# talmolab/track-mjx

Measured on AMD Instinct MI355X. Metric: env-steps/sec (whole node), rodent task @ 4096 envs/GPU, higher is better.
Workload: dtype f32

## Files before the change

### include/tmjx.h

```cpp
#ifndef TMJX_H
#define TMJX_H
#include <stddef.h>
#include <stdint.h>

#ifdef __cplusplus
extern "C" {
#endif

#define TMJX_OK 0
#define TMJX_EINVAL (-22)
#define TMJX_ENOMEM (-12)
#define TMJX_EHIP (-5)

typedef struct tmjx_model tmjx_model;

typedef struct tmjx_layout_t {
  int32_t nq, nv, nu, nbody, ncon, nefc, obs_size, ref_obs_size, n_metrics, window;
  int32_t qpos, qvel, act, qacc_warmstart, time;
  int32_t xpos, xmat_torso, qfrc_actuator;
  int32_t prev_ctrl, action_buffer, done, steps_f;
  int32_t first_phys, first_obs, first_prev_ctrl;
  int32_t state_rows;
  int32_t i_clip_idx, i_start_frame, i_buffer_index, i_nan_count, istate_rows;
  int32_t ws_rows;
// ... 42 lines not shown
int tmjx_gae(const float *truncation, const float *termination, const float *rewards, const float *values,
             const float *bootstrap, float lambda_, float discount, float *vs, float *advantages, int T, int B,
             void *stream);

typedef struct {
  int32_t T, B, A, Z;
  float reward_scaling, discounting, gae_lambda, clip_eps, entropy_cost, kl_weight;
  int32_t normalize_advantage;
  int32_t accumulate;
} tmjx_ppo_cfg_t;
int tmjx_ppo_scratch_floats(int T, int B);
int tmjx_ppo_loss(const tmjx_ppo_cfg_t *cfg, const float *logits, const float *raw_action, const float *behaviour_logp,
                  const float *noise, const float *baseline, const float *bootstrap, const float *reward, const float *discount,
                  const float *truncation, const float *fc2, float *dlogits, float *dbaseline, float *dfc2, float *scratch,
                  float *out, void *stream);

#define TMJX_PPO_PHASE_A 1
#define TMJX_PPO_PHASE_B 2
#define TMJX_PPO_PHASE_C 4
#define TMJX_PPO_PHASE_D 8
int tmjx_ppo_loss_phases(const tmjx_ppo_cfg_t *cfg, const float *logits, const float *raw_action, const float *behaviour_logp,
                         const float *noise, const float *baseline, const float *bootstrap, const float *reward, const float *discount,
                         const float *truncation, const float *fc2, float *dlogits, float *dbaseline, float *dfc2, float *scratch,
                         float *out, int phases, void *stream);

int tmjx_silu_ln_partial_floats(int rows, int H);
int tmjx_silu_ln_fwd(const float *z, const float *bias, const float *gamma, const float *beta, float *y, float *stats, int rows, int H,
                     float eps, void *stream);
int tmjx_silu_ln_bwd(const float *dy, const float *z, const float *bias, const float *gamma, const float *stats, float *dz, float *grads,
                     float *partial, int rows, int H, void *stream);
int tmjx_silu_ln_fwd_bf16(const float *z, const float *bias, const float *gamma, const float *beta, uint16_t *y16, int ldy16, float *stats, int rows, int H,
                          float eps, void *stream);
int tmjx_silu_ln_bwd_bf16(const float *dy, const float *z, const float *bias, const float *gamma, const float *stats, uint16_t *dz16, int lddz16, float *grads,
                          float *partial, int rows, int H, void *stream);

int tmjx_gather_normalize(const float *src, const int64_t *idx, const float *mean, const float *std, float *out, int T, int R, int B,
                          int W, void *stream);
int tmjx_gather_minibatch(const float *obs, const float *next_last, const float *raw_action, const float *log_prob, const float *reward, const float *discount,
                          const float *truncation, const int64_t *idx, const float *mean, const float *std, float *obs_n, float *next_n, float *raw_action_g,
                          float *scalars_g, int T, int R, int B, int W, int A, void *stream);
#define TMJX_MINIBATCH_STATE_WORDS (16 + 16 * 64)
typedef struct tmjx_minibatch_t {
  const float *obs, *next_last, *raw_action, *log_prob, *reward, *discount, *truncation;
  const int64_t *perm;
  const float *mean, *std;
  float *obs_n, *next_n, *raw_action_g, *scalars_g;
  float *eps, *noise;
  int64_t *state;
  uint64_t seed;
  int32_t T, R, B, W, A, Z, advance;
} tmjx_minibatch_t;
int tmjx_minibatch_begin(const tmjx_minibatch_t *mb, void *stream);
int tmjx_minibatch_begin_bf16(const tmjx_minibatch_t *mb, uint16_t *obs_n16, int ld16, void *stream);
int tmjx_philox4x32_10(const uint32_t *ctr_key_dev, uint32_t *out_dev, void *stream);

int tmjx_latent_concat_bwd(const float *dx, const float *eps, const float *fc2, float *dfc2, int n, int Z, int dx_stride, void *stream);
int tmjx_latent_concat_bwd_add(const float *dx, const float *eps, const float *fc2, const float *add, float *dfc2, int n, int Z, int dx_stride,
                               void *stream);

int tmjx_latent_concat(const float *fc2, const float *eps, const float *obs, float *x, int n, int Z, int obs_w, int ref_w,
                       int64_t obs_s0, int64_t obs_s1, const float *mean, const float *std, int x_stride, uint64_t seed, const int64_t *rng_state,
                       void *stream);
int tmjx_sample_action(const float *logits, const float *noise, float *raw, float *action_t, float *logp, int n, int A, uint64_t seed,
                       int64_t *rng_state, void *stream);

int tmjx_linear_act_ok(const float *A, int64_t lda, const float *W, int ldw, int K);
int tmjx_linear_act(const float *A, int64_t lda, const float *W, int ldw, const float *bias, float *C, int M, int N, int K,
                    const float *mean, const float *inv_std, void *stream);
int tmjx_linear_nolds(const float *A, int64_t sa_row, int64_t sa_k, const float *W, const float *bias, float *C, int M, int N, int K,
                      void *stream);
int tmjx_linear_nolds_norm(const float *A, int64_t sa_row, int64_t sa_k, const float *W, const float *bias, float *C, int M, int N, int K,
                           const float *mean, const float *inv_std, void *stream);

int tmjx_linear_nolds_bf16(const float *A, int64_t sa_row, int64_t sa_k, const uint16_t *W, int ldw, const float *bias, float *C, int M, int N, int K,
                           const float *mean, const float *inv_std, void *stream);

int tmjx_colsum_scratch_floats(int width);
int tmjx_colsum(const float *src, float *out, float *scratch, int rows, int width, void *stream);

typedef struct tmjx_colsum_problem_t { const float *partial; float *out; int32_t rows, width; } tmjx_colsum_problem_t;
int tmjx_colsum_grouped(const tmjx_colsum_problem_t *problems, int n, void *stream);

int tmjx_adam_clip(float *param, const float *grad, float *exp_avg, float *exp_avg_sq, const float *grad_norm, long long n, float lr,
                   float beta1, float beta2, float eps, float bias_correction1, float bias_correction2, float max_norm, void *stream);
int tmjx_adam_norm_floats(void);
int tmjx_adam_clip_norm(float *param, const float *grad, float *exp_avg, float *exp_avg_sq, float *norm_scratch, float *norm_out, long long n, float lr,
                        float beta1, float beta2, float eps, float bias_correction1, float bias_correction2, float max_norm, void *stream);
int tmjx_adam_clip_norm_frozen(float *param, const float *grad, float *exp_avg, float *exp_avg_sq, float *norm_scratch, float *norm_out, long long n,
                               long long frozen_lo, long long frozen_hi, float lr, float beta1, float beta2, float eps, float bias_correction1,
                               float bias_correction2, float max_norm, void *stream);

int tmjx_gemm_nt(const float *A, int lda, const float *W, int ldw, const float *bias, float *C, int ldc, int M, int N, int K, void *stream);
int tmjx_gemm_nn(const float *A, int lda, const float *W, int ldw, float *C, int ldc, int M, int N, int K, void *stream);
int tmjx_gemm_nt_silu_ln_ok(const float *A, int lda, const float *W, int ldw, int N);
int tmjx_gemm_nt_silu_ln(const float *A, int lda, const float *W, int ldw, const float *bias, const float *gamma, const float *beta, float *Z, float *Y,
                         int ldc, float *stats, int M, int N, int K, float eps, void *stream);
int tmjx_gemm_nn_ln_bwd_ok(const float *dY, int ldy, const float *W, int ldw, int N);
long long tmjx_gemm_nn_ln_bwd_partial_floats(int M, int N);
int tmjx_gemm_nn_ln_bwd(const float *dY, int ldy, const float *W, int ldw, const float *z, const float *bias, const float *gamma, const float *stats,
                        float *dz, float *partial, int M, int N, int K, void *stream);
int tmjx_gemm_nt_silu_ok(const float *A, int lda, const float *W, int ldw);
int tmjx_gemm_nt_silu(const float *A, int lda, const float *W, int ldw, const float *bias, float *Z, float *Y, int ldc, int M, int N, int K, void *stream);
int tmjx_silu_fwd(const float *z, const float *bias, float *y, long long rows, int N, void *stream);
int tmjx_silu_bwd(const float *dy, const float *z, const float *bias, float *dz, long long rows, int N, void *stream);
int tmjx_gemm_nn_silu_bwd_ok(const float *dY, int ldy, const float *W, int ldw);
int tmjx_gemm_nn_silu_bwd(const float *dY, int ldy, const float *W, int ldw, const float *z, const float *bias, float *dZ, int M, int N, int K, void *stream);
// ... 323 lines not shown
```

### track_mjx_amd/csrc/ppo_kernels.h

```cpp
#pragma once
#include "silu_math.h"
#include "act_shared.h"
#include <hip/hip_runtime.h>
#include <math.h>

struct PpoCfg {
  int T, B, A, Z;
  float reward_scaling, discounting, gae_lambda, clip_eps, entropy_cost, kl_weight;
  int normalize_advantage;
  int accumulate;
};

#define PPO_BLOCK 256
#define PPO_ALPHA 0.95f
__device__ __forceinline__ float ppo_sigmoid(float x) { return 1.f / (1.f + expf(-x)); }

template <int NV>
__device__ __forceinline__ void ppo_block_sum(float *v, float *lds) {
  const int tid = threadIdx.x, lane = tid & 63, w = tid >> 6, nw = (blockDim.x + 63) >> 6;
#pragma unroll
  for (int k = 0; k < NV; k++) {
    float x = v[k];
    for (int off = 32; off >= 1; off >>= 1) x += __shfl_xor(x, off);
    if (lane == 0) lds[k * 16 + w] = x;
// ... 668 lines not shown
  const size_t q_eps = g.eps ? ((size_t)g.T * g.B * g.Z + 3) / 4 : 0, q_noise = g.noise ? (n_act + 3) / 4 : 0;
  const size_t e0 = n_obs + n_next, e1 = e0 + n_act, e2 = e1 + n_sc, e3 = e2 + q_eps, total = e3 + q_noise;
  for (size_t i = (size_t)blockIdx.x * 256 + threadIdx.x; i < total; i += (size_t)gridDim.x * 256) {
    if (i < e0) {
      const bool nx = i >= n_obs;
      const size_t j = nx ? i - n_obs : i;
      const int c = (int)(j % w4);
      const size_t tb = j / w4;
      const int b = (int)(tb % g.B), t = (int)(tb / g.B);
      const float *src = nx ? g.next_last : g.obs;
      const float4 v = reinterpret_cast<const float4 *>(src + ((size_t)t * g.R + (size_t)idx[b]) * g.W)[c];
      const float4 m = reinterpret_cast<const float4 *>(g.mean)[c], s = reinterpret_cast<const float4 *>(g.stdv)[c];
      const float4 o = {(v.x - m.x) / s.x, (v.y - m.y) / s.y, (v.z - m.z) / s.z, (v.w - m.w) / s.w};
      reinterpret_cast<float4 *>((nx ? g.next_n : g.obs_n) + tb * g.W)[c] = o;
      if (!nx && g.obs_n16) *reinterpret_cast<uint2 *>(g.obs_n16 + tb * g.ld16 + 4 * c) = uint2{silu_ln_pack(o.x, o.y), silu_ln_pack(o.z, o.w)};
    } else if (i < e1) {
      const size_t j = i - e0;
      const int c = (int)(j % g.A);
      const size_t tb = j / g.A;
      const int b = (int)(tb % g.B), t = (int)(tb / g.B);
      g.raw_action_g[j] = g.raw_action[((size_t)t * g.R + (size_t)idx[b]) * g.A + c];
    } else if (i < e2) {
      const size_t j = i - e1;
      const int b = (int)(j % g.B);
      const size_t kt = j / g.B;
      const int t = (int)(kt % g.T), k = (int)(kt / g.T);
      g.scalars_g[j] = g.scalar[k][(size_t)t * g.R + (size_t)idx[b]];
    } else {
      const bool second = i >= e3;
      const size_t q = second ? i - e3 : i - e2, n = second ? n_act : (size_t)g.T * g.B * g.Z;
      float v[4];
      tm_normal4(g.seed, ctr, second ? 1u : 0u, (unsigned)q, v);
      float *dst = second ? g.noise : g.eps;
#pragma unroll
      for (int k = 0; k < 4; k++) if (4 * q + k < n) dst[4 * q + k] = v[k];
    }
  }
  if (g.state && g.advance) {
    __syncthreads();
    if (threadIdx.x == 0) {
      const unsigned sub = blockIdx.x % TM_MB_SUBTICKETS, nsub = min((unsigned)gridDim.x, (unsigned)TM_MB_SUBTICKETS);
      const unsigned members = (gridDim.x - sub + TM_MB_SUBTICKETS - 1) / TM_MB_SUBTICKETS;
      unsigned long long *st = (unsigned long long *)g.state, *subt = st + TM_MB_STATE_HEAD + (size_t)TM_MB_STATE_STRIDE * sub;
      if (__hip_atomic_fetch_add(subt, 1ull, __ATOMIC_RELAXED, __HIP_MEMORY_SCOPE_AGENT) == (unsigned long long)members - 1ull) {
        __hip_atomic_store(subt, 0ull, __ATOMIC_RELAXED, __HIP_MEMORY_SCOPE_AGENT);
        if (__hip_atomic_fetch_add(st + 2, 1ull, __ATOMIC_RELAXED, __HIP_MEMORY_SCOPE_AGENT) == (unsigned long long)nsub - 1ull) {
          __hip_atomic_store(st + 2, 0ull, __ATOMIC_RELAXED, __HIP_MEMORY_SCOPE_AGENT);
          g.state[0] += 1; g.state[1] += 1;
        }
      }
    }
  }
}
__global__ void k_philox_kat(const unsigned *ctr_key, unsigned *out) {
  if (threadIdx.x == 0) tm_philox4x32_10(ctr_key[0], ctr_key[1], ctr_key[2], ctr_key[3], ctr_key[4], ctr_key[5], out);
}

__global__ __launch_bounds__(256) void k_latent_concat(const float *__restrict__ fc2, const float *__restrict__ eps, const float *__restrict__ obs,
                                                       float *__restrict__ x, int n, int Z, int obs_w, int ref_w, long long obs_s0, long long obs_s1,
                                                       const float *__restrict__ mean, const float *__restrict__ stdv, int x_stride,
                                                       unsigned long long seed, const long long *__restrict__ rng_state) {
  TM_PRIO_ACTING();
  const int W = Z + obs_w - ref_w;
  const unsigned long long ctr = rng_state ? (unsigned long long)rng_state[0] : 0ull;
  for (size_t i = (size_t)blockIdx.x * blockDim.x + threadIdx.x; i < (size_t)n * x_stride; i += (size_t)gridDim.x * blockDim.x) {
    int c = (int)(i % x_stride); size_t e = i / x_stride;
    float v = 0.f;
    if (c < Z) {
      v = tm_latent_sample(tm_normal_at(eps, seed, ctr, 2u, e * Z + c), fc2[e * 2 * Z + Z + c], fc2[e * 2 * Z + c]);
    } else if (c < W) { int k = ref_w + c - Z; v = obs[(long long)e * obs_s0 + (long long)k * obs_s1]; if (mean) v = tm_obs_normalised(v, mean[k], stdv[k]); }
    x[e * (size_t)x_stride + c] = v;
  }
}
__global__ __launch_bounds__(256) void k_latent_concat_bwd(const float *__restrict__ dx, const float *__restrict__ eps, const float *__restrict__ fc2,
                                                           float *__restrict__ dfc2, int n, int Z, int dx_stride, const float *__restrict__ add) {
  for (size_t i = (size_t)blockIdx.x * 256 + threadIdx.x; i < (size_t)n * Z; i += (size_t)gridDim.x * 256) {
    int c = (int)(i % Z); size_t e = i / Z;
    float g = dx[e * (size_t)dx_stride + c];
    float gm = g, gv = g * eps[e * Z + c] * (0.5f * expf(0.5f * fc2[e * 2 * Z + Z + c]));
    if (add) { gm = add[e * 2 * Z + c] + gm; gv = add[e * 2 * Z + Z + c] + gv; }
    dfc2[e * 2 * Z + c] = gm;
    dfc2[e * 2 * Z + Z + c] = gv;
  }
}
__global__ __launch_bounds__(PPO_BLOCK) void k_sample_action(const float *__restrict__ logits, const float *__restrict__ noise, float *__restrict__ raw,
                                                             float *__restrict__ action_t, float *__restrict__ logp, int n, int A,
                                                             unsigned long long seed, long long *__restrict__ rng_state) {
  TM_PRIO_ACTING();
  const int gid = blockIdx.x * blockDim.x + threadIdx.x, e = gid / PPO_G, sub = gid % PPO_G;
  const unsigned long long ctr = rng_state ? (unsigned long long)rng_state[0] : 0ull;
  float lp = 0.f;
  if (e < n) lp = sample_action_lane(logits + (size_t)e * 2 * A, noise, raw, action_t, n, A, (size_t)e, sub, seed, ctr);
  lp = ppo_group_sum(lp);
  if (e < n && sub == 0) logp[e] = lp;
  if (rng_state) {
    __syncthreads();
    if (threadIdx.x == 0) {
      unsigned long long *st = (unsigned long long *)rng_state;
      if (__hip_atomic_fetch_add(st + 1, 1ull, __ATOMIC_RELAXED, __HIP_MEMORY_SCOPE_AGENT) == (unsigned long long)gridDim.x - 1ull) {
        __hip_atomic_store(st + 1, 0ull, __ATOMIC_RELAXED, __HIP_MEMORY_SCOPE_AGENT);
        rng_state[0] += 1;
      }
    }
  }
}

// ... 375 lines not shown
```

### track_mjx_amd/csrc/tmjx_hip.hip

```cpp
#include <hip/hip_runtime.h>

#include <stdlib.h>

#include <string>
#include <vector>

#include "../../include/tmjx.h"
#include "env_core.h"
#include "host_launch.h"
#include "model_host.h"
#include "wave_physics.h"
#ifdef TMJX_LANE_IMPL
#include "../../tests/lane/physics_core.h"
#endif

struct tmjx_model {
  DModel h;
  DModel *d = nullptr;
  float *clips[7] = {nullptr, nullptr, nullptr, nullptr, nullptr, nullptr, nullptr};
  int block = 64;
  int wave = 1;
  bool rodent = false;
  mutable float *mspill = nullptr;
  mutable int mspill_envs = 0;
// ... 708 lines not shown
  switch (H) { case 64: TMJX_FWD(1); break; case 128: TMJX_FWD(2); break; case 256: TMJX_FWD(4); break; case 512: TMJX_FWD(8); break;
               case 1024: TMJX_FWD(16); break; default: return fail(TMJX_EINVAL, "H must be 64, 128, 256, 512 or 1024"); }
#undef TMJX_FWD
  return check_launch("k_silu_ln_fwd");
}
int tmjx_silu_ln_fwd(const float *z, const float *bias, const float *gamma, const float *beta, float *y, float *stats, int rows, int H,
                     float eps, void *stream) {
  if (!y) return fail(TMJX_EINVAL, "null argument");
  return silu_ln_fwd_any(z, bias, gamma, beta, y, nullptr, 0, stats, rows, H, eps, stream);
}
int tmjx_silu_ln_fwd_bf16(const float *z, const float *bias, const float *gamma, const float *beta, uint16_t *y16, int ldy16, float *stats, int rows, int H,
                          float eps, void *stream) {
  if (!y16) return fail(TMJX_EINVAL, "null argument");
  return silu_ln_fwd_any(z, bias, gamma, beta, nullptr, y16, ldy16, stats, rows, H, eps, stream);
}

static int silu_ln_bwd_any(const float *dy, const float *z, const float *bias, const float *gamma, const float *stats, float *dz, uint16_t *dz16, int lddz16, float *grads,
                           float *partial, int rows, int H, void *stream) {
  if (!dy || !z || !bias || !gamma || !stats || (!dz && !dz16) || !grads || !partial) return fail(TMJX_EINVAL, "null argument");
  if (rows < 1) return fail(TMJX_EINVAL, "rows must be >= 1");
  if (dz16 && (lddz16 < H || (lddz16 & 3) || ((uintptr_t)dz16 & 7))) return fail(TMJX_EINVAL, "tmjx_silu_ln_bwd_bf16: the output's rows must be 8-byte aligned and H wide");
  hipStream_t s = (hipStream_t)stream;
  const int nblk = (rows + BLK_ROWS_PER_BLOCK - 1) / BLK_ROWS_PER_BLOCK;
  unsigned short *o16 = (unsigned short *)dz16;
#define TMJX_BWD(V) do { if (o16) hipLaunchKernelGGL((k_silu_ln_bwd<V, true>), dim3(nblk), dim3(256), 0, s, dy, z, bias, gamma, stats, dz, partial, rows, o16, lddz16); \
                         else hipLaunchKernelGGL((k_silu_ln_bwd<V, false>), dim3(nblk), dim3(256), 0, s, dy, z, bias, gamma, stats, dz, partial, rows, o16, 0); } while (0)
  switch (H) { case 64: TMJX_BWD(1); break; case 128: TMJX_BWD(2); break; case 256: TMJX_BWD(4); break; case 512: TMJX_BWD(8); break;
               case 1024: TMJX_BWD(16); break; default: return fail(TMJX_EINVAL, "H must be 64, 128, 256, 512 or 1024"); }
#undef TMJX_BWD
  hipLaunchKernelGGL(k_colsum, dim3((3 * H + 31) / 32), dim3(256), 0, s, (const float *)partial, grads, nblk, 3 * H);
  return check_launch("k_silu_ln_bwd");
}
int tmjx_silu_ln_bwd(const float *dy, const float *z, const float *bias, const float *gamma, const float *stats, float *dz, float *grads,
                     float *partial, int rows, int H, void *stream) {
  if (!dz) return fail(TMJX_EINVAL, "null argument");
  return silu_ln_bwd_any(dy, z, bias, gamma, stats, dz, nullptr, 0, grads, partial, rows, H, stream);
}
int tmjx_silu_ln_bwd_bf16(const float *dy, const float *z, const float *bias, const float *gamma, const float *stats, uint16_t *dz16, int lddz16, float *grads,
                          float *partial, int rows, int H, void *stream) {
  if (!dz16) return fail(TMJX_EINVAL, "null argument");
  return silu_ln_bwd_any(dy, z, bias, gamma, stats, nullptr, dz16, lddz16, grads, partial, rows, H, stream);
}

int tmjx_gather_normalize(const float *src, const int64_t *idx, const float *mean, const float *std, float *out, int T, int R, int B,
                          int W, void *stream) {
  if (!src || !idx || !mean || !std || !out) return fail(TMJX_EINVAL, "null argument");
  if (T < 1 || R < 1 || B < 1 || W < 4 || (W & 3)) return fail(TMJX_EINVAL, "bad T / R / B / W (W must be a multiple of 4)");
  size_t total = (size_t)T * B * (W >> 2);
  int grid = (int)((total + 255) / 256 < 8192 ? (total + 255) / 256 : 8192);
  hipLaunchKernelGGL(k_gather_normalize, dim3(grid), dim3(256), 0, (hipStream_t)stream, src, (const long long *)idx, mean, std, out, T, R, B, W);
  return check_launch("k_gather_normalize");
}

static int launch_minibatch(const MinibatchGather &g, hipStream_t s) {
  if (!g.obs || !g.next_last || !g.raw_action || !g.scalar[0] || !g.scalar[1] || !g.scalar[2] || !g.scalar[3] || !g.idx || !g.mean || !g.stdv || !g.obs_n || !g.next_n ||
      !g.raw_action_g || !g.scalars_g)
    return fail(TMJX_EINVAL, "null argument");
  if (g.T < 1 || g.R < 1 || g.B < 1 || g.A < 1 || g.W < 4 || (g.W & 3)) return fail(TMJX_EINVAL, "bad T / R / B / A / W (W must be a multiple of 4)");
  if (g.eps && g.Z < 1) return fail(TMJX_EINVAL, "Z must be >= 1 with eps");
  const size_t nact = (size_t)g.T * g.B * g.A;
  const size_t total = (size_t)g.T * g.B * (g.W >> 2) + (size_t)g.B * (g.W >> 2) + nact + (size_t)4 * g.T * g.B + (g.eps ? ((size_t)g.T * g.B * g.Z + 3) / 4 : 0) +
                       (g.noise ? (nact + 3) / 4 : 0);
  const int grid = (int)((total + 255) / 256 < 8192 ? (total + 255) / 256 : 8192);
  hipLaunchKernelGGL(k_gather_minibatch, dim3(grid), dim3(256), 0, s, g);
  return check_launch("k_gather_minibatch");
}
int tmjx_gather_minibatch(const float *obs, const float *next_last, const float *raw_action, const float *log_prob, const float *reward, const float *discount,
                          const float *truncation, const int64_t *idx, const float *mean, const float *std, float *obs_n, float *next_n, float *raw_action_g,
                          float *scalars_g, int T, int R, int B, int W, int A, void *stream) {
  MinibatchGather g{obs, next_last, raw_action, {log_prob, reward, discount, truncation}, (const long long *)idx, mean, std, obs_n, next_n, raw_action_g, scalars_g,
                    nullptr, nullptr, nullptr, 0ull, T, R, B, W, A, 0, 0, nullptr, 0};
  return launch_minibatch(g, (hipStream_t)stream);
}
int tmjx_minibatch_begin(const tmjx_minibatch_t *m, void *stream) {
  if (!m) return fail(TMJX_EINVAL, "null argument");
  if ((m->eps || m->noise || m->advance) && !m->state) return fail(TMJX_EINVAL, "tmjx_minibatch_begin: draws / advance need the device state");
  MinibatchGather g{m->obs, m->next_last, m->raw_action, {m->log_prob, m->reward, m->discount, m->truncation}, (const long long *)m->perm, m->mean, m->std, m->obs_n,
                    m->next_n, m->raw_action_g, m->scalars_g, m->eps, m->noise, (long long *)m->state, (unsigned long long)m->seed, m->T, m->R, m->B, m->W, m->A,
                    m->Z, m->advance, nullptr, 0};
  return launch_minibatch(g, (hipStream_t)stream);
}
int tmjx_minibatch_begin_bf16(const tmjx_minibatch_t *m, uint16_t *obs_n16, int ld16, void *stream) {
  if (!m || !obs_n16) return fail(TMJX_EINVAL, "null argument");
  if ((m->eps || m->noise || m->advance) && !m->state) return fail(TMJX_EINVAL, "tmjx_minibatch_begin_bf16: draws / advance need the device state");
  if (ld16 < m->W || (ld16 & 3) || ((uintptr_t)obs_n16 & 7)) return fail(TMJX_EINVAL, "tmjx_minibatch_begin_bf16: the twin's rows must be 8-byte aligned and W wide");
  MinibatchGather g{m->obs, m->next_last, m->raw_action, {m->log_prob, m->reward, m->discount, m->truncation}, (const long long *)m->perm, m->mean, m->std, m->obs_n,
                    m->next_n, m->raw_action_g, m->scalars_g, m->eps, m->noise, (long long *)m->state, (unsigned long long)m->seed, m->T, m->R, m->B, m->W, m->A,
                    m->Z, m->advance, (unsigned short *)obs_n16, ld16};
  return launch_minibatch(g, (hipStream_t)stream);
}
int tmjx_philox4x32_10(const uint32_t *ctr_key_dev, uint32_t *out_dev, void *stream) {
  if (!ctr_key_dev || !out_dev) return fail(TMJX_EINVAL, "null argument");
  hipLaunchKernelGGL(k_philox_kat, dim3(1), dim3(64), 0, (hipStream_t)stream, ctr_key_dev, out_dev);
  return check_launch("k_philox_kat");
}

int tmjx_colsum_scratch_floats(int width) { return COLSUM_CHUNKS * width; }

int tmjx_colsum(const float *src, float *out, float *scratch, int rows, int width, void *stream) {
  if (!src || !out || !scratch) return fail(TMJX_EINVAL, "null argument");
  if (rows < 1 || width < 1) return fail(TMJX_EINVAL, "rows and width must be >= 1");
  hipStream_t s = (hipStream_t)stream;
  hipLaunchKernelGGL(k_colsum_rows, dim3((width + 31) / 32, COLSUM_CHUNKS), dim3(256), 0, s, src, scratch, rows, width);
  hipLaunchKernelGGL(k_colsum, dim3((width + 31) / 32), dim3(256), 0, s, (const float *)scratch, out, COLSUM_CHUNKS, width);
  return check_launch("k_colsum_rows");
}

int tmjx_colsum_grouped(const tmjx_colsum_problem_t *q, int n, void *stream) {
  if (!q || n < 1 || n > COLSUM_GROUP_MAX) return fail(TMJX_EINVAL, "tmjx_colsum_grouped: 1 .. 16 problems");
  ColsumGroup G;
  G.n = n;
  int blocks = 0;
  for (int i = 0; i < n; i++) {
    if (!q[i].partial || !q[i].out || q[i].rows < 1 || q[i].width < 1) return fail(TMJX_EINVAL, "tmjx_colsum_grouped: bad problem");
    G.p[i] = ColsumProblem{q[i].partial, q[i].out, q[i].rows, q[i].width, blocks};
    blocks += (q[i].width + 31) / 32;
  }
  hipLaunchKernelGGL(k_colsum_grouped, dim3(blocks), dim3(256), 0, (hipStream_t)stream, G);
  return check_launch("k_colsum_grouped");
}

int tmjx_adam_clip(float *param, const float *grad, float *exp_avg, float *exp_avg_sq, const float *grad_norm, long long n, float lr,
                   float beta1, float beta2, float eps, float bias_correction1, float bias_correction2, float max_norm, void *stream) {
  if (!param || !grad || !exp_avg || !exp_avg_sq || !grad_norm) return fail(TMJX_EINVAL, "null argument");
  if (n < 1 || !(bias_correction1 > 0.f) || !(bias_correction2 > 0.f) || !(max_norm > 0.f)) return fail(TMJX_EINVAL, "bad n / bias corrections / max_norm");
  int grid = (int)((n + 255) / 256 < 4096 ? (n + 255) / 256 : 4096);
  hipLaunchKernelGGL(k_adam_clip<false>, dim3(grid), dim3(256), 0, (hipStream_t)stream, param, grad, exp_avg, exp_avg_sq, grad_norm, n, lr, beta1, beta2, eps,
                     bias_correction1, bias_correction2, max_norm, (float *)nullptr);
  return check_launch("k_adam_clip");
}
int tmjx_adam_norm_floats(void) { return ADAM_NORM_PARTS; }
int tmjx_adam_clip_norm(float *param, const float *grad, float *exp_avg, float *exp_avg_sq, float *norm_scratch, float *norm_out, long long n, float lr,
                        float beta1, float beta2, float eps, float bias_correction1, float bias_correction2, float max_norm, void *stream) {
  if (!param || !grad || !exp_avg || !exp_avg_sq || !norm_scratch) return fail(TMJX_EINVAL, "null argument");
  if (n < 1 || !(bias_correction1 > 0.f) || !(bias_correction2 > 0.f) || !(max_norm > 0.f)) return fail(TMJX_EINVAL, "bad n / bias corrections / max_norm");
  if ((uintptr_t)grad & 15) return fail(TMJX_EINVAL, "tmjx_adam_clip_norm: the gradient buffer must be 16-byte aligned");
  hipStream_t s = (hipStream_t)stream;
  hipLaunchKernelGGL(k_grad_sumsq, dim3(ADAM_NORM_PARTS), dim3(256), 0, s, grad, n, norm_scratch);
  int grid = (int)((n + 255) / 256 < 4096 ? (n + 255) / 256 : 4096);
  hipLaunchKernelGGL(k_adam_clip<true>, dim3(grid), dim3(256), 0, s, param, grad, exp_avg, exp_avg_sq, (const float *)norm_scratch, n, lr, beta1, beta2, eps,
                     bias_correction1, bias_correction2, max_norm, norm_out);
  return check_launch("k_adam_clip(norm)");
// ... 437 lines not shown
```

### track_mjx_amd/hip.py

```python
from __future__ import annotations

import ctypes as C
import os
import subprocess
from pathlib import Path

_PKG = Path(__file__).resolve().parent
SO_PATH = Path(os.environ.get("TMJX_SO", str(_PKG / "libtmjx_hip.so")))
CSRC = _PKG / "csrc"
SOURCES = (CSRC / "tmjx_hip.hip", CSRC / "tmjx_bf16.hip", CSRC / "tmjx_wave.hip", CSRC / "tmjx_chain.hip", CSRC / "tmjx_lstm.hip",
           CSRC / "tmjx_rollout.hip", CSRC / "tmjx_wave_sensors.hip", CSRC / "tmjx_wave_align.hip", CSRC / "tmjx_wave_rand.hip", CSRC / "tmjx_render.hip", CSRC / "tmjx_act.hip", CSRC / "tmjx_pca.hip", CSRC / "tmjx_pca_wide.hip", CSRC / "tmjx_readout.hip", CSRC / "tmjx_intervene.hip", CSRC / "tmjx_kmeans.hip", CSRC / "tmjx_hmm.hip", CSRC / "tmjx_spectrogram.hip", CSRC / "tmjx_arhmm.hip")
SOURCE_FLAGS = {"tmjx_wave.hip": ("-mllvm", "-disable-machine-licm"),
                "tmjx_wave_sensors.hip": ("-mllvm", "-disable-machine-licm"),
                "tmjx_wave_rand.hip": ("-mllvm", "-disable-machine-licm")}


class TmjxError(RuntimeError):
    pass


class Layout(C.Structure):
    _fields_ = [(n, C.c_int32) for n in (
        "nq", "nv", "nu", "nbody", "ncon", "nefc", "obs_size", "ref_obs_size", "n_metrics", "window",
        "qpos", "qvel", "act", "qacc_warmstart", "time", "xpos", "xmat_torso", "qfrc_actuator",
# ... 146 lines not shown

class ArhmmInfo(C.Structure):
    _fields_ = HmmInfo._fields_ + [("n_singular", C.c_int32), ("pad_", C.c_int32)]


INTERVENE_SUBSPACE, INTERVENE_UNITS, INTERVENE_MAX_W, INTERVENE_MAX_K = 0, 1, 1024, 16


class Intervene(C.Structure):
    _fields_ = [("h", C.c_void_p), ("ld", C.c_int32), ("w", C.c_int32), ("n", C.c_int32), ("mode", C.c_int32), ("dirs", C.c_void_p), ("K", C.c_int32),
                ("ldv", C.c_int32), ("center", C.c_void_p), ("gain", C.c_void_p), ("offset", C.c_void_p), ("dose", C.c_void_p), ("t_on", C.c_void_p),
                ("t_off", C.c_void_p), ("proj", C.c_void_p), ("ldp", C.c_int32), ("pad_", C.c_int32)]


class PcaInfo(C.Structure):
    _fields_ = [("sweeps", C.c_int32), ("converged", C.c_int32), ("off_rel", C.c_float), ("moments_ms", C.c_float), ("jacobi_ms", C.c_float)]


class StripStyle(C.Structure):
    _fields_ = [(k, C.c_int32) for k in ("margin_left", "margin_right", "margin_top", "margin_bottom")] + \
               [("line_half_width", C.c_float), ("marker_radius", C.c_float), ("colour", (C.c_uint8 * 4) * 8)] + \
               [(k, C.c_uint8 * 4) for k in ("background", "axes", "terminated")]


class PpoCfg(C.Structure):
    _fields_ = [("T", C.c_int32), ("B", C.c_int32), ("A", C.c_int32), ("Z", C.c_int32), ("reward_scaling", C.c_float),
                ("discounting", C.c_float), ("gae_lambda", C.c_float), ("clip_eps", C.c_float), ("entropy_cost", C.c_float),
                ("kl_weight", C.c_float), ("normalize_advantage", C.c_int32), ("accumulate", C.c_int32)]


_i, _i64, _u64, _f, _d, _vp, _s, _P = C.c_int, C.c_int64, C.c_uint64, C.c_float, C.c_double, C.c_void_p, C.c_char_p, C.POINTER
SIGNATURES = {
    "tmjx_model_create": ([_s, C.c_size_t, _P(_vp)], _i),
    "tmjx_model_destroy": ([_vp], None),
    "tmjx_layout": ([_vp, _P(Layout)], _i),
    "tmjx_clips_upload": ([_vp] * 6 + [_i, _i], _i),
    "tmjx_reset": ([_vp] * 9 + [_i, _vp], _i),
    "tmjx_step": ([_vp] * 10 + [_i, _vp], _i),
    "tmjx_physics": ([_vp, _vp, _vp, _i, _vp, _i, _vp], _i),
    "tmjx_physics_step": ([_vp] * 4 + [_i, _vp], _i),
    "tmjx_forward": ([_vp, _vp, _vp, _i, _vp], _i),
    "tmjx_reward_obs": ([_vp] * 10 + [_i, _vp], _i),
    "tmjx_reward_frame": ([_vp] * 14 + [_i, _vp], _i),
    "tmjx_gae": ([_vp] * 5 + [_f, _f, _vp, _vp, _i, _i, _vp], _i),
    "tmjx_ppo_scratch_floats": ([_i, _i], _i),
    "tmjx_ppo_loss": ([_P(PpoCfg)] + [_vp] * 16, _i),
    "tmjx_ppo_loss_phases": ([_P(PpoCfg)] + [_vp] * 15 + [_i, _vp], _i),
    "tmjx_silu_ln_partial_floats": ([_i, _i], _i),
    "tmjx_silu_ln_fwd": ([_vp] * 6 + [_i, _i, _f, _vp], _i),
    "tmjx_silu_ln_bwd": ([_vp] * 8 + [_i, _i, _vp], _i),
    "tmjx_silu_ln_fwd_bf16": ([_vp] * 5 + [_i, _vp, _i, _i, _f, _vp], _i),
    "tmjx_silu_ln_bwd_bf16": ([_vp] * 6 + [_i, _vp, _vp, _i, _i, _vp], _i),
    "tmjx_minibatch_begin_bf16": ([_P(Minibatch), _vp, _i, _vp], _i),
    "tmjx_gather_normalize": ([_vp] * 5 + [_i] * 4 + [_vp], _i),
    "tmjx_latent_concat": ([_vp] * 4 + [_i] * 4 + [_i64, _i64, _vp, _vp, _i, _u64, _vp, _vp], _i),
    "tmjx_latent_concat_bwd": ([_vp] * 4 + [_i, _i, _i, _vp], _i),
    "tmjx_latent_concat_bwd_add": ([_vp] * 5 + [_i, _i, _i, _vp], _i),
    "tmjx_sample_action": ([_vp] * 5 + [_i, _i, _u64, _vp, _vp], _i),
    "tmjx_linear_nolds": ([_vp, _i64, _i64, _vp, _vp, _vp, _i, _i, _i, _vp], _i),
    "tmjx_linear_act": ([_vp, _i64, _vp, _i, _vp, _vp, _i, _i, _i, _vp, _vp, _vp], _i),
    "tmjx_linear_act_ok": ([_vp, _i64, _vp, _i, _i], _i),
    "tmjx_linear_nolds_norm": ([_vp, _i64, _i64, _vp, _vp, _vp, _i, _i, _i, _vp, _vp, _vp], _i),
    "tmjx_linear_nolds_bf16": ([_vp, _i64, _i64, _vp, _i, _vp, _vp, _i, _i, _i, _vp, _vp, _vp], _i),
    "tmjx_adam_clip": ([_vp] * 5 + [_i64] + [_f] * 7 + [_vp], _i),
    "tmjx_adam_clip_norm": ([_vp] * 6 + [_i64] + [_f] * 7 + [_vp], _i),
    "tmjx_adam_clip_norm_frozen": ([_vp] * 6 + [_i64, _i64, _i64] + [_f] * 7 + [_vp], _i),
    "tmjx_adam_norm_floats": ([], _i),
    "tmjx_colsum_scratch_floats": ([_i], _i),
    "tmjx_colsum": ([_vp, _vp, _vp, _i, _i, _vp], _i),
    "tmjx_gather_minibatch": ([_vp] * 14 + [_i] * 5 + [_vp], _i),
    "tmjx_minibatch_begin": ([_P(Minibatch), _vp], _i),
    "tmjx_philox4x32_10": ([_vp, _vp, _vp], _i),
    "tmjx_gemm_nt": ([_vp, _i, _vp, _i, _vp, _vp] + [_i] * 4 + [_vp], _i),
    "tmjx_gemm_nt_silu_ln": ([_vp, _i, _vp, _i] + [_vp] * 5 + [_i, _vp, _i, _i, _i, _f, _vp], _i),
    "tmjx_gemm_nt_silu_ln_ok": ([_vp, _i, _vp, _i, _i], _i),
    "tmjx_gemm_nn": ([_vp, _i, _vp, _i, _vp] + [_i] * 4 + [_vp], _i),
    "tmjx_colsum_grouped": ([_P(ColsumProblem), _i, _vp], _i),
    "tmjx_gemm_nn_ln_bwd": ([_vp, _i, _vp, _i] + [_vp] * 6 + [_i, _i, _i, _vp], _i),
    "tmjx_gemm_nn_ln_bwd_ok": ([_vp, _i, _vp, _i, _i], _i),
    "tmjx_gemm_nn_ln_bwd_partial_floats": ([_i, _i], _i64),
    "tmjx_gemm_dw": ([_vp, _i, _vp, _i, _vp, _vp, _vp, _i, _i, _i, _vp], _i),
    "tmjx_gemm_dw_grouped": ([_P(DwProblem), _i, _vp], _i),
    "tmjx_gemm_dw_scratch_floats": ([_i, _i, _i], _i64),
    "tmjx_set_wrappers": ([_vp, _i, _i], _i),
    "tmjx_set_action_repeat": ([_vp, _i], _i),
    "tmjx_stats_scratch_floats": ([_i], _i),
    "tmjx_stats_sums": ([_vp] * 4 + [_i64, _i, _vp], _i),
    "tmjx_stats_apply": ([_vp, _f] + [_vp] * 4 + [_i, _f, _f, _vp], _i),
    "tmjx_stats_apply_pinned": ([_vp, _f] + [_vp] * 4 + [_i, _i, _f, _f, _vp], _i),
    "tmjx_rollout_store": ([_P(RolloutStore), _vp], _i),
    "tmjx_clips_share": ([_vp, _vp], _i),
    "tmjx_gemm_nt_silu": ([_vp, _i, _vp, _i, _vp, _vp, _vp] + [_i] * 4 + [_vp], _i),
    "tmjx_gemm_nt_silu_ok": ([_vp, _i, _vp, _i], _i),
    "tmjx_silu_fwd": ([_vp, _vp, _vp, _i64, _i, _vp], _i),
    "tmjx_silu_bwd": ([_vp] * 4 + [_i64, _i, _vp], _i),
    "tmjx_gemm_nn_silu_bwd_ok": ([_vp, _i, _vp, _i], _i),
    "tmjx_gemm_nn_silu_bwd": ([_vp, _i, _vp, _i, _vp, _vp, _vp, _i, _i, _i, _vp], _i),
    "tmjx_silu_bwd_rank1": ([_vp] * 5 + [_i64, _i, _vp], _i),
    "tmjx_head_dw_scratch_floats": ([_i, _i], _i64),
    "tmjx_head_dw": ([_vp, _vp, _i, _vp, _vp, _vp, _i, _i, _vp], _i),
    "tmjx_head_fwd_ok": ([_vp, _i, _vp, _i], _i),
    "tmjx_head_fwd": ([_vp, _i, _vp, _vp, _vp, _i, _i, _vp], _i),
    "tmjx_bf16_shadow": ([_P(Bf16Shadow), _i, _vp], _i),
    "tmjx_bgemm_nt": ([_vp, _i, _i, _vp, _i, _vp, _vp] + [_i] * 4 + [_vp], _i),
    "tmjx_bgemm_dw": ([_vp, _i, _i, _vp, _i, _i, _vp, _i, _vp, _vp, _i, _i, _i, _vp], _i),
    "tmjx_bgemm_dw_grouped": ([_P(BdwProblem), _i, _i, _vp], _i),
# ... 190 lines not shown
```

Before: 1.724 million.

## Gather minibatch rows with one wave per row instead of flat element grid

```diff
diff --git a/include/tmjx.h b/include/tmjx.h
--- a/include/tmjx.h
+++ b/include/tmjx.h
@@ -118,6 +118,7 @@
 } tmjx_minibatch_t;
 int tmjx_minibatch_begin(const tmjx_minibatch_t *mb, void *stream);
 int tmjx_minibatch_begin_bf16(const tmjx_minibatch_t *mb, uint16_t *obs_n16, int ld16, void *stream);
+int tmjx_minibatch_begin_flat(const tmjx_minibatch_t *mb, uint16_t *obs_n16, int ld16, void *stream);
 int tmjx_philox4x32_10(const uint32_t *ctr_key_dev, uint32_t *out_dev, void *stream);
 
 int tmjx_latent_concat_bwd(const float *dx, const float *eps, const float *fc2, float *dfc2, int n, int Z, int dx_stride, void *stream);
diff --git a/track_mjx_amd/csrc/ppo_kernels.h b/track_mjx_amd/csrc/ppo_kernels.h
--- a/track_mjx_amd/csrc/ppo_kernels.h
+++ b/track_mjx_amd/csrc/ppo_kernels.h
@@ -744,6 +744,93 @@
     }
   }
 }
+#define TM_MB_ROWS_PER_WAVE 1
+#define TM_MB_ROWS_PER_BLOCK (4 * TM_MB_ROWS_PER_WAVE)
+#define TM_MB_SMALL_PER_BLOCK 1024
+__global__ __launch_bounds__(256) void k_minibatch_rows(MinibatchGather g, unsigned small_blocks) {
+  const unsigned w4 = (unsigned)g.W >> 2, T = (unsigned)g.T, B = (unsigned)g.B, A = (unsigned)g.A;
+  const unsigned long long ctr = g.state ? (unsigned long long)g.state[0] : 0ull;
+  const long long *idx = g.idx + (g.state ? g.state[1] * (long long)g.B : 0ll);
+  if (blockIdx.x >= small_blocks) {
+    const unsigned wave = (blockIdx.x - small_blocks) * 4u + (threadIdx.x >> 6), lane = threadIdx.x & 63u, n_rows = T * B, all_rows = n_rows + B;
+    const unsigned n_waves = (gridDim.x - small_blocks) * 4u;
+    const float4 *src[TM_MB_ROWS_PER_WAVE];
+    float4 *dst[TM_MB_ROWS_PER_WAVE];
+    unsigned short *d16[TM_MB_ROWS_PER_WAVE];
+    bool on[TM_MB_ROWS_PER_WAVE];
+#pragma unroll
+    for (unsigned r = 0; r < TM_MB_ROWS_PER_WAVE; r++) {
+      const unsigned row = wave + r * n_waves;
+      on[r] = row < all_rows;
+      const bool nx = row >= n_rows;
+      const unsigned tb = !on[r] ? 0u : nx ? row - n_rows : row, t = tb / B, b = tb - t * B;
+      src[r] = reinterpret_cast<const float4 *>((nx ? g.next_last : g.obs) + ((size_t)t * g.R + (size_t)idx[b]) * g.W);
+      dst[r] = reinterpret_cast<float4 *>((nx ? g.next_n : g.obs_n) + (size_t)tb * g.W);
+      d16[r] = (!nx && g.obs_n16) ? g.obs_n16 + (size_t)tb * g.ld16 : nullptr;
+    }
+    for (unsigned c0 = lane; c0 < w4; c0 += 256u) {
+      float4 v[TM_MB_ROWS_PER_WAVE][4];
+#pragma unroll
+      for (unsigned r = 0; r < TM_MB_ROWS_PER_WAVE; r++)
+#pragma unroll
+        for (unsigned k = 0; k < 4; k++) if (on[r] && c0 + 64u * k < w4) v[r][k] = src[r][c0 + 64u * k];
+#pragma unroll
+      for (unsigned k = 0; k < 4; k++) {
+        const unsigned c = c0 + 64u * k;
+        if (c < w4) {
+          const float4 m = reinterpret_cast<const float4 *>(g.mean)[c], s = reinterpret_cast<const float4 *>(g.stdv)[c];
+#pragma unroll
+          for (unsigned r = 0; r < TM_MB_ROWS_PER_WAVE; r++) {
+            if (on[r]) {
+              const float4 o = {(v[r][k].x - m.x) / s.x, (v[r][k].y - m.y) / s.y, (v[r][k].z - m.z) / s.z, (v[r][k].w - m.w) / s.w};
+              dst[r][c] = o;
+              if (d16[r]) *reinterpret_cast<uint2 *>(d16[r] + 4u * c) = uint2{silu_ln_pack(o.x, o.y), silu_ln_pack(o.z, o.w)};
+            }
+          }
+        }
+      }
+    }
+  } else {
+    const unsigned n_act = T * B * A, n_sc = 4u * T * B, n_z = T * B * (unsigned)g.Z;
+    const unsigned q_eps = g.eps ? (n_z + 3u) / 4u : 0u, q_noise = g.noise ? (n_act + 3u) / 4u : 0u;
+    const unsigned e1 = n_act, e2 = e1 + n_sc, e3 = e2 + q_eps, total = e3 + q_noise;
+#pragma unroll
+    for (unsigned u = 0; u < TM_MB_SMALL_PER_BLOCK / 256; u++) {
+      const unsigned i = blockIdx.x * TM_MB_SMALL_PER_BLOCK + 256u * u + threadIdx.x;
+      if (i >= total) break;
+      if (i < e1) {
+        const unsigned tb = i / A, c = i - tb * A, t = tb / B, b = tb - t * B;
+        g.raw_action_g[i] = g.raw_action[((size_t)t * g.R + (size_t)idx[b]) * g.A + c];
+      } else if (i < e2) {
+        const unsigned j = i - e1, kt = j / B, b = j - kt * B, k = kt / T, t = kt - k * T;
+        g.scalars_g[j] = g.scalar[k][(size_t)t * g.R + (size_t)idx[b]];
+      } else {
+        const bool second = i >= e3;
+        const unsigned q = second ? i - e3 : i - e2, n = second ? n_act : n_z;
+        float v[4];
+        tm_normal4(g.seed, ctr, second ? 1u : 0u, q, v);
+        float *dst = second ? g.noise : g.eps;
+#pragma unroll
+        for (unsigned k = 0; k < 4; k++) if (4u * q + k < n) dst[4u * q + k] = v[k];
+      }
+    }
+  }
+  if (g.state && g.advance) {
+    __syncthreads();
+    if (threadIdx.x == 0) {
+      const unsigned sub = blockIdx.x % TM_MB_SUBTICKETS, nsub = min((unsigned)gridDim.x, (unsigned)TM_MB_SUBTICKETS);
+      const unsigned members = (gridDim.x - sub + TM_MB_SUBTICKETS - 1) / TM_MB_SUBTICKETS;
+      unsigned long long *st = (unsigned long long *)g.state, *subt = st + TM_MB_STATE_HEAD + (size_t)TM_MB_STATE_STRIDE * sub;
+      if (__hip_atomic_fetch_add(subt, 1ull, __ATOMIC_RELAXED, __HIP_MEMORY_SCOPE_AGENT) == (unsigned long long)members - 1ull) {
+        __hip_atomic_store(subt, 0ull, __ATOMIC_RELAXED, __HIP_MEMORY_SCOPE_AGENT);
+        if (__hip_atomic_fetch_add(st + 2, 1ull, __ATOMIC_RELAXED, __HIP_MEMORY_SCOPE_AGENT) == (unsigned long long)nsub - 1ull) {
+          __hip_atomic_store(st + 2, 0ull, __ATOMIC_RELAXED, __HIP_MEMORY_SCOPE_AGENT);
+          g.state[0] += 1; g.state[1] += 1;
+        }
+      }
+    }
+  }
+}
 __global__ void k_philox_kat(const unsigned *ctr_key, unsigned *out) {
   if (threadIdx.x == 0) tm_philox4x32_10(ctr_key[0], ctr_key[1], ctr_key[2], ctr_key[3], ctr_key[4], ctr_key[5], out);
 }
diff --git a/track_mjx_amd/csrc/tmjx_hip.hip b/track_mjx_amd/csrc/tmjx_hip.hip
--- a/track_mjx_amd/csrc/tmjx_hip.hip
+++ b/track_mjx_amd/csrc/tmjx_hip.hip
@@ -784,18 +784,26 @@
   return check_launch("k_gather_normalize");
 }
 
-static int launch_minibatch(const MinibatchGather &g, hipStream_t s) {
+static int launch_minibatch(const MinibatchGather &g, hipStream_t s, bool flat = false) {
   if (!g.obs || !g.next_last || !g.raw_action || !g.scalar[0] || !g.scalar[1] || !g.scalar[2] || !g.scalar[3] || !g.idx || !g.mean || !g.stdv || !g.obs_n || !g.next_n ||
       !g.raw_action_g || !g.scalars_g)
     return fail(TMJX_EINVAL, "null argument");
   if (g.T < 1 || g.R < 1 || g.B < 1 || g.A < 1 || g.W < 4 || (g.W & 3)) return fail(TMJX_EINVAL, "bad T / R / B / A / W (W must be a multiple of 4)");
   if (g.eps && g.Z < 1) return fail(TMJX_EINVAL, "Z must be >= 1 with eps");
   const size_t nact = (size_t)g.T * g.B * g.A;
-  const size_t total = (size_t)g.T * g.B * (g.W >> 2) + (size_t)g.B * (g.W >> 2) + nact + (size_t)4 * g.T * g.B + (g.eps ? ((size_t)g.T * g.B * g.Z + 3) / 4 : 0) +
-                       (g.noise ? (nact + 3) / 4 : 0);
-  const int grid = (int)((total + 255) / 256 < 8192 ? (total + 255) / 256 : 8192);
-  hipLaunchKernelGGL(k_gather_minibatch, dim3(grid), dim3(256), 0, s, g);
-  return check_launch("k_gather_minibatch");
+  const size_t small = nact + (size_t)4 * g.T * g.B + (g.eps ? ((size_t)g.T * g.B * g.Z + 3) / 4 : 0) + (g.noise ? (nact + 3) / 4 : 0);
+  if (flat) {
+    const size_t total = (size_t)g.T * g.B * (g.W >> 2) + (size_t)g.B * (g.W >> 2) + small;
+    const int grid = (int)((total + 255) / 256 < 8192 ? (total + 255) / 256 : 8192);
+    hipLaunchKernelGGL(k_gather_minibatch, dim3(grid), dim3(256), 0, s, g);
+    return check_launch("k_gather_minibatch");
+  }
+  const size_t rows = (size_t)g.T * g.B + g.B, lim = 0x7fffffffull;
+  if (rows > lim || nact > lim || (size_t)g.T * g.B * (g.Z > 0 ? g.Z : 0) > lim || small > lim)
+    return fail(TMJX_EINVAL, "minibatch too large: T B + B rows, T B A, T B Z and the small leaves together must each stay below 2^31");
+  const size_t small_blocks = (small + TM_MB_SMALL_PER_BLOCK - 1) / TM_MB_SMALL_PER_BLOCK, row_blocks = (rows + TM_MB_ROWS_PER_BLOCK - 1) / TM_MB_ROWS_PER_BLOCK;
+  hipLaunchKernelGGL(k_minibatch_rows, dim3((unsigned)(small_blocks + row_blocks)), dim3(256), 0, s, g, (unsigned)small_blocks);
+  return check_launch("k_minibatch_rows");
 }
 int tmjx_gather_minibatch(const float *obs, const float *next_last, const float *raw_action, const float *log_prob, const float *reward, const float *discount,
                           const float *truncation, const int64_t *idx, const float *mean, const float *std, float *obs_n, float *next_n, float *raw_action_g,
@@ -820,6 +828,15 @@
                     m->next_n, m->raw_action_g, m->scalars_g, m->eps, m->noise, (long long *)m->state, (unsigned long long)m->seed, m->T, m->R, m->B, m->W, m->A,
                     m->Z, m->advance, (unsigned short *)obs_n16, ld16};
   return launch_minibatch(g, (hipStream_t)stream);
+}
+int tmjx_minibatch_begin_flat(const tmjx_minibatch_t *m, uint16_t *obs_n16, int ld16, void *stream) {
+  if (!m) return fail(TMJX_EINVAL, "null argument");
+  if ((m->eps || m->noise || m->advance) && !m->state) return fail(TMJX_EINVAL, "tmjx_minibatch_begin_flat: draws / advance need the device state");
+  if (obs_n16 && (ld16 < m->W || (ld16 & 3) || ((uintptr_t)obs_n16 & 7))) return fail(TMJX_EINVAL, "tmjx_minibatch_begin_flat: the twin's rows must be 8-byte aligned and W wide");
+  MinibatchGather g{m->obs, m->next_last, m->raw_action, {m->log_prob, m->reward, m->discount, m->truncation}, (const long long *)m->perm, m->mean, m->std, m->obs_n,
+                    m->next_n, m->raw_action_g, m->scalars_g, m->eps, m->noise, (long long *)m->state, (unsigned long long)m->seed, m->T, m->R, m->B, m->W, m->A,
+                    m->Z, m->advance, (unsigned short *)obs_n16, obs_n16 ? ld16 : 0};
+  return launch_minibatch(g, (hipStream_t)stream, true);
 }
 int tmjx_philox4x32_10(const uint32_t *ctr_key_dev, uint32_t *out_dev, void *stream) {
   if (!ctr_key_dev || !out_dev) return fail(TMJX_EINVAL, "null argument");
diff --git a/track_mjx_amd/hip.py b/track_mjx_amd/hip.py
--- a/track_mjx_amd/hip.py
+++ b/track_mjx_amd/hip.py
@@ -222,6 +222,7 @@
     "tmjx_silu_ln_fwd_bf16": ([_vp] * 5 + [_i, _vp, _i, _i, _f, _vp], _i),
     "tmjx_silu_ln_bwd_bf16": ([_vp] * 6 + [_i, _vp, _vp, _i, _i, _vp], _i),
     "tmjx_minibatch_begin_bf16": ([_P(Minibatch), _vp, _i, _vp], _i),
+    "tmjx_minibatch_begin_flat": ([_P(Minibatch), _vp, _i, _vp], _i),
     "tmjx_gather_normalize": ([_vp] * 5 + [_i] * 4 + [_vp], _i),
     "tmjx_latent_concat": ([_vp] * 4 + [_i] * 4 + [_i64, _i64, _vp, _vp, _i, _u64, _vp, _vp], _i),
     "tmjx_latent_concat_bwd": ([_vp] * 4 + [_i, _i, _i, _vp], _i),
```

New measurement: 1.727 million, median of 6. About the same (+0.2%).
